# ACMMM2021-Anonymous/video-graph-ssl

Hardware: AMD Instinct MI355X
Metric: pretrain_clips_per_sec (higher is better)
Workload: dtype bf16x6 (fp32 tensors; conv products as 6 bf16 MFMAs on hi/mid/lo splits = fp32-grade, fp32 accumulate; everything else fp32)

## Files before the change

video-graph-ssl_amd/_hip.py:

```python
import ctypes as C
import os

import torch

_HERE = os.path.dirname(os.path.abspath(__file__))
LIB_PATH = os.environ.get('GCA_LIB_PATH') or os.path.join(_HERE, 'libgca_hip.so')


class HipLibraryMissing(RuntimeError):
    pass


if not os.path.exists(LIB_PATH):
    raise HipLibraryMissing(
        'libgca_hip.so is not built (%s). Run ./build_hip.sh or __graft_entry__.build(); there is no '
        'CPU fallback for the product path.' % LIB_PATH)
lib = C.CDLL(LIB_PATH)

c_i32, c_i64, c_f32, c_f64, c_vp = C.c_int32, C.c_int64, C.c_float, C.c_double, C.c_void_p


class ConvGeom(C.Structure):
    _fields_ = [(n, c_i32) for n in ('N', 'C', 'D', 'H', 'W', 'K', 'kd', 'kh', 'kw', 'sd', 'sh', 'sw',
                                     'pd', 'ph', 'pw', 'OD', 'OH', 'OW')] + [('x_batch_stride', c_i64)] + \
# ... 71 lines not shown
                                  c_f32, c_vp, c_vp, c_vp]),
    'gca_graph_gcn_fwd': (c_i32, [c_vp, c_vp, c_i64, c_i64, c_i64, c_i64, c_vp, c_vp]),
    'gca_graph_gcn_bwd_ws_bytes': (c_i64, [c_i64, c_i64, c_i64, c_i64]),
    'gca_graph_gcn_bwd': (c_i32, [c_vp, c_vp, c_vp, c_i64, c_i64, c_i64, c_i64, c_vp, c_vp, c_vp, c_vp]),
    'gca_ema_update': (c_i32, [c_vp, c_vp, c_i64, c_f32, c_vp]),
    'gca_ema_update_dev': (c_i32, [c_vp, c_vp, c_i64, c_vp, c_vp]),
    'gca_sgd_step': (c_i32, [c_vp, c_vp, c_vp, c_i64, c_vp, c_vp, c_f32, c_f32, c_i32, c_i32, c_vp, c_vp]),
    'gca_lars_job_chunks': (c_i32, []),
    'gca_lars_step': (c_i32, [c_vp, c_vp, c_vp, c_i64, c_vp, c_vp, c_vp, c_i64, c_vp, c_vp, c_i64, c_vp, c_vp, c_vp, c_vp, c_f32,
                              c_i32, c_f64, c_f64, c_vp, c_vp]),
    'gca_adam_step': (c_i32, [c_vp, c_vp, c_vp, c_vp, c_i64, c_vp, c_vp, c_f64, c_f64, c_f64, c_i32, c_vp, c_vp, c_vp]),
    'gca_adam_advance': (c_i32, [c_vp, c_vp, c_vp]),
    'gca_grad_clip_ws_bytes': (c_i64, []),
    'gca_grad_clip_coef': (c_i32, [c_vp, c_i64, c_f32, c_vp, c_vp, c_vp]),
    'gca_conv_wgrad_partial': (c_i32, [_GP, c_vp, c_vp, c_vp, c_vp, c_vp, c_vp, c_vp, c_vp]),
    'gca_conv_xf_ok': (c_i32, [_GP]),
    'gca_conv_fwd_xf': (c_i32, [_GP, c_vp, c_vp, c_vp, c_vp, c_vp, c_vp, c_vp, c_vp, c_vp, c_vp, c_vp]),
    'gca_conv_wgrad_xf': (c_i32, [_GP, c_vp, c_vp, c_vp, c_vp, c_vp, c_vp, c_i32, c_vp, c_vp]),
    'gca_conv_fwd_slabs': (c_i32, [_GP, c_vp, c_vp, c_vp, c_vp, c_vp, c_vp]),
    'gca_bn_train_fwd_slabs': (c_i32, [c_vp, c_i64, c_f64, c_vp, c_vp, c_f32, c_f32, c_vp, c_vp, c_vp, c_vp, c_vp, c_vp, c_vp, c_vp,
                                       c_vp, c_i32, c_i64, c_i64, c_i64, c_vp, c_i64, c_vp]),
    'gca_conv_dzf_ok': (c_i32, [_GP]),
    'gca_conv_wgrad_dzf': (c_i32, [_GP, c_vp, c_vp, c_vp, c_vp, c_i32, c_vp, c_vp, c_i32, c_vp, c_vp]),
    'gca_conv_wgrad_dzf_partial': (c_i32, [_GP, c_vp, c_vp, c_vp, c_vp, c_i32, c_vp, c_vp, c_vp, c_vp]),
    'gca_bn_bwd_consts_elems': (c_i64, [c_i64]),
    'gca_bn_bwd_sums': (c_i32, [c_vp, c_vp, c_vp, c_vp, c_vp, c_i32, c_i64, c_i64, c_i64, c_vp, c_vp, c_i64, c_vp, c_vp, c_vp,
                                c_vp, c_i32, c_vp]),
    'gca_reduce_jobs_finalize_host': (c_i64, [c_vp, c_i64]),
    'gca_splitk_reduce_batched': (c_i32, [c_vp, c_i64, c_i64, c_vp]),
    'gca_clip_prepare': (c_i32, [c_vp, c_i64, c_i64, c_i64, c_i64, c_i64, c_vp, c_vp, c_vp, c_i64, c_i64, c_vp, c_i32, c_vp]),
    'gca_clip_augment_ws_bytes': (c_i64, [c_i64, c_i64, c_i64]),
    'gca_clip_augment': (c_i32, [c_vp, c_i64, c_i64, c_i64, c_i64, c_i64, c_vp, c_vp, c_vp, c_vp, c_vp, c_vp, c_vp, c_i64, c_i64,
                                 c_vp, c_i32, c_vp, c_vp]),
    'gca_clip_views': (c_i32, [c_vp, c_i64, c_i64, c_i64, c_i64, c_vp, c_vp, c_i64, c_vp, c_i64, c_i64, c_i64, c_vp, c_vp, c_i64, c_i64,
                               c_i64, c_vp, c_vp]),
    'gca_retrieval_ws_bytes': (c_i64, [c_i64, c_i64, c_i64, c_i32, c_i32]),
    'gca_retrieval_topk': (c_i32, [c_vp, c_vp, c_i64, c_i64, c_i64, c_i32, c_i32, c_vp, c_vp, c_i32, c_vp, c_vp, c_vp, c_vp,
                                   c_i64, c_vp]),
    'gca_knn_vote': (c_i32, [c_vp, c_vp, c_i64, c_i32, c_i32, c_vp, c_i64, c_vp, c_i64, c_i64, c_i32, c_f32, c_vp, c_vp, c_vp,
                             c_vp]),
    'gca_ntxent_ws_bytes': (c_i64, [c_i64, c_i64]),
    'gca_ntxent_path': (c_i32, [c_i64, c_i64, c_i32, c_vp, c_vp]),
    'gca_ntxent_fwd': (c_i32, [c_vp, c_i64, c_i64, c_f32, c_vp, c_vp, c_vp, c_vp, c_vp, c_vp]),
    'gca_ntxent_bwd': (c_i32, [c_vp, c_vp, c_i64, c_i64, c_f32, c_vp, c_f32, c_vp, c_vp, c_vp]),
    'gca_barlow_ws_bytes': (c_i64, [c_i64, c_i64]),
    'gca_barlow_fwd': (c_i32, [c_vp, c_vp, c_i64, c_i64, c_f32, c_f32, c_vp, c_vp, c_vp, c_vp, c_vp, c_vp]),
    'gca_barlow_bwd': (c_i32, [c_vp, c_vp, c_vp, c_vp, c_vp, c_i64, c_i64, c_f32, c_vp, c_f32, c_vp, c_vp, c_vp, c_vp]),
    'gca_vicreg_ws_bytes': (c_i64, [c_i64, c_i64]),
    'gca_vicreg_fwd': (c_i32, [c_vp, c_vp, c_i64, c_i64, c_f32, c_f32, c_f32, c_f32, c_vp, c_vp, c_vp, c_vp, c_vp]),
    'gca_vicreg_bwd': (c_i32, [c_vp, c_vp, c_vp, c_vp, c_i64, c_i64, c_f32, c_f32, c_f32, c_vp, c_f32, c_vp, c_vp, c_vp, c_vp]),
    'gca_rows_normalize': (c_i32, [c_vp, c_i64, c_i64, c_vp]),
    'gca_swav_ws_bytes': (c_i64, [c_i64, c_i64, c_i64]),
    'gca_swav_fwd': (c_i32, [c_vp, c_vp, c_vp, c_i64, c_i64, c_i64, c_f32, c_f32, c_i64, c_vp, c_vp, c_vp, c_vp, c_vp]),
    'gca_swav_dz_splits': (c_i32, [c_i64, c_i64, c_i64]),
    'gca_swav_bwd': (c_i32, [c_vp, c_vp, c_vp, c_vp, c_i64, c_i64, c_i64, c_vp, c_f32, c_vp, c_vp, c_vp, c_i32, c_vp, c_vp]),
    'gca_dino_ws_bytes': (c_i64, [c_i64, c_i64, c_i64]),
    'gca_dino_fwd': (c_i32, [c_vp, c_vp, c_vp, c_vp, c_vp, c_vp, c_i64, c_i64, c_i64, c_f32, c_vp, c_f32, c_vp, c_i32, c_vp, c_vp, c_vp,
                             c_vp, c_vp]),
    'gca_dino_fwd_grid': (c_i32, [c_vp, c_vp, c_vp, c_vp, c_vp, c_vp, c_i64, c_i64, c_i64, c_f32, c_vp, c_f32, c_vp, c_i32, c_vp, c_vp,
                                  c_vp, c_i32, c_vp, c_vp]),
    'gca_classifier_ws_bytes': (c_i64, [c_i64, c_i64, c_i64]),
    'gca_classifier_fwd': (c_i32, [c_vp, c_vp, c_vp, c_vp, c_i64, c_i64, c_i64, c_vp, c_vp, c_vp, c_vp, c_vp, c_i64, c_vp]),
    'gca_classifier_bwd': (c_i32, [c_vp, c_vp, c_vp, c_vp, c_vp, c_vp, c_f32, c_i64, c_i64, c_i64, c_vp, c_vp, c_i32, c_vp, c_i32,
                                   c_vp, c_i64, c_vp]),
    'gca_rank_ge': (c_i32, [c_vp, c_vp, c_i64, c_i64, c_vp, c_vp]),
    'gca_grad_unscale_clip': (c_i32, [c_vp, c_i64, c_f32, c_vp, c_f32, c_f32, c_i32, c_f32, c_vp, c_vp, c_vp]),
    'gca_scale_dev': (c_i32, [c_vp, c_i64, c_vp, c_f32, c_vp]),
    'gca_fill': (c_i32, [c_vp, c_i64, c_f32, c_vp]),
    'gca_axpy': (c_i32, [c_vp, c_vp, c_i64, c_f32, c_vp]),
    'gca_scale': (c_i32, [c_vp, c_i64, c_f32, c_vp]),
    'gca_axpy_f16': (c_i32, [c_vp, c_vp, c_i64, c_f32, c_vp]),
    'gca_cast_f16': (c_i32, [c_vp, c_i64, c_i64, c_i64, c_vp, c_vp]),
    'gca_conv_pack_jobs_host': (c_i64, [_GP, c_i32, c_vp, c_vp, c_vp]),
    'gca_conv_pack_jobs_finalize_host': (c_i64, [c_vp, c_i64]),
    'gca_conv_pack_batched': (c_i32, [c_vp, c_i64, c_i64, c_vp]),
    'gca_gather_rows': (c_i32, [c_vp, c_vp, c_i64, c_i64, c_i64, c_vp, c_vp]),
}
for _name, (_res, _args) in SIGNATURES.items():
    _fn = getattr(lib, _name)
    _fn.restype, _fn.argtypes = _res, _args


PACK_JOB_BYTES = 128


class ReduceJob(C.Structure):
    _fields_ = [('slabs', C.c_void_p), ('dw', C.c_void_p), ('n', C.c_int64), ('splits', C.c_int32), ('accumulate', C.c_int32),
                ('first_block', C.c_int32), ('nblocks', C.c_int32)]


def ptr(t, half_ok=False):
    if t is None:
        return None
    if not t.is_cuda:
        raise RuntimeError('gca HIP ops need tensors on the GPU (got %s); there is no CPU fallback' % t.device)
    if t.dtype is not torch.float32 and not (half_ok and t.dtype is torch.float16) and t.is_floating_point():
        raise TypeError('this gca HIP op has no %s kernel' % t.dtype)
    return t.data_ptr()


def aptr(t):
    return ptr(t, True)


def is_half(*ts):
    kinds = {t.dtype for t in ts if t is not None}
    if len(kinds) > 1:
        raise TypeError('mixed activation storage types: %s' % sorted(map(str, kinds)))
    return int(kinds == {torch.float16})


def stream():
    return torch.cuda.current_stream().cuda_stream


def check(rc, what):
    if rc != 0:
        raise RuntimeError('%s failed with status %d (%s)' % (what, rc, {-1: 'invalid argument', -2: 'launch error'}.get(rc, '?')))


def call(name, *args):
    check(getattr(lib, name)(*args), name)
```

video-graph-ssl_amd/csrc/conv3d.hip:

```cpp
#include <cstring>
#include <type_traits>
#include "conv_halo.h"

#include <cstdlib>
#include <vector>

using namespace gca_conv;

namespace {

constexpr int LDK = BK + 4;
constexpr int lds_pitch(int math) { return math == 2 ? 28 : (math == 3 ? 12 : LDK); }
constexpr int lds_bufs(int tm, bool vec, int math) { return (math >= 1 || vec || tm >= 4) ? 1 : 2; }
constexpr int cmax(int a, int b) { return a > b ? a : b; }

template <int TM, int BN, int FAST, bool VEC, int MATH, bool H = false>
__device__ __forceinline__ void igemm_tile(
    const void* __restrict__ src, const float* __restrict__ apack, const int2* __restrict__ table,
    const float* __restrict__ bias, void* __restrict__ dst, float* __restrict__ psum,
    float* __restrict__ psq, float* __restrict__ slab, const IgemmParams p, int bid,
    float* __restrict__ As_, float* __restrict__ Bs_, int* __restrict__ taptab) {
  constexpr unsigned ES = H ? 2u : 4u;
  constexpr int BM = 32 * TM, TN = BN / 128;
  constexpr int A_F4 = (BM * 4 + 255) / 256;
// ... 585 lines not shown
                                      gca_xcd_remap((int)blockIdx.x - nA, (int)gridDim.x - nA), As_, Bs_, taptab);
  }
}

__device__ __forceinline__ int class_of(const int* __restrict__ first, int id) {
  int ci = 0;
#pragma unroll
  for (int i = 1; i < MAX_MERGED_CLASSES; ++i) ci += id >= first[i] ? 1 : 0;
  return ci;
}

template <int TM, int BN, int FAST, bool VEC, int MATH, bool H = false>
__global__ __launch_bounds__(256) void conv_igemm_classes_kernel(
    const void* __restrict__ src, const float* __restrict__ apack, const int2* __restrict__ table, void* __restrict__ dst,
    float* __restrict__ slab, const ClassBlock cb) {
  __shared__ __attribute__((aligned(16))) float As_[lds_bufs(TM, VEC, MATH) * 32 * TM * lds_pitch(MATH)];
  __shared__ __attribute__((aligned(16))) float Bs_[lds_bufs(TM, VEC, MATH) * BN * lds_pitch(MATH)];
  __shared__ int taptab[64];
  const int ci = class_of(cb.first_wg, (int)blockIdx.x);
  const int first = cb.first_wg[ci], count = cb.first_wg[ci + 1] - first;
  igemm_tile<TM, BN, FAST, VEC, MATH, H>(src, apack + cb.pack_off[ci], table + cb.table_off[ci], nullptr, dst, nullptr, nullptr,
                                         slab + cb.slab_off[ci], cb.p[ci], gca_xcd_remap((int)blockIdx.x - first, count), As_, Bs_,
                                         taptab);
}

constexpr int FINISH_CHUNK = 1024;
template <typename T>
__device__ __forceinline__ void splitk_finish_part(
    const float* __restrict__ slab, int splits, const float* __restrict__ bias, T* __restrict__ dst,
    float* __restrict__ psum, float* __restrict__ psq, const IgemmParams& p, int m, int part, int P, double* sh) {
  const float b = bias ? bias[m] : 0.f;
  const long long lo = (long long)part * FINISH_CHUNK;
  long long hi = lo + FINISH_CHUNK; if (hi > p.Ntot) hi = p.Ntot;
  const int QSP = p.QD * p.QH * p.QW, QHW = p.QH * p.QW, DHW = p.DH * p.DW;
  const long long DSP = (long long)p.DD * DHW;
  double s = 0.0, q = 0.0;
  for (long long n = lo + threadIdx.x; n < hi; n += 256) {
    float v = 0.f;
    const float* sp0 = slab + (long long)m * p.Ntot + n;
    const long long sstride = (long long)p.DK * p.Ntot;
    int k = 0;
    for (; k + 4 <= splits; k += 4) {
      const float l0 = sp0[(long long)k * sstride], l1 = sp0[(long long)(k + 1) * sstride];
      const float l2 = sp0[(long long)(k + 2) * sstride], l3 = sp0[(long long)(k + 3) * sstride];
      v += l0; v += l1; v += l2; v += l3;
    }
    for (; k < splits; ++k) v += sp0[(long long)k * sstride];
    s += (double)v; q += (double)v * (double)v;
    v += b;
    const int img = (int)(n / QSP);
    const int sp = (int)(n - (long long)img * QSP);
    const int qd = sp / QHW, rr = sp - qd * QHW;
    const int qh = rr / p.QW, qw = rr - qh * p.QW;
    const long long dsp = (long long)(qd * p.dm_d + p.do_d) * DHW + (qh * p.dm_h + p.do_h) * p.DW + (qw * p.dm_w + p.do_w);
    T* d = dst + ((long long)img * p.DK + m) * DSP + dsp;
    if (p.accumulate) v += (float)*d;
    *d = (T)v;
  }
  if (psum) {
    s = gca_block_sum256_d(s, sh);
    q = gca_block_sum256_d(q, sh);
    if (threadIdx.x == 0) { psum[(long long)m * P + part] = (float)s; psq[(long long)m * P + part] = (float)q; }
  }
}

template <typename T>
__global__ __launch_bounds__(256) void conv_splitk_finish_kernel(
    const float* __restrict__ slab, int splits, const float* __restrict__ bias, T* __restrict__ dst,
    float* __restrict__ psum, float* __restrict__ psq, IgemmParams p) {
  __shared__ double sh[4];
  splitk_finish_part<T>(slab, splits, bias, dst, psum, psq, p, blockIdx.x, blockIdx.y, gridDim.y, sh);
}

template <typename T>
__global__ __launch_bounds__(256) void conv_splitk_finish_classes_kernel(const float* __restrict__ slab, T* __restrict__ dst,
                                                                         const ClassBlock cb) {
  __shared__ double sh[4];
  const int ci = class_of(cb.first_part, (int)blockIdx.y);
  const int first = cb.first_part[ci];
  splitk_finish_part<T>(slab + cb.slab_off[ci], cb.p[ci].splits, nullptr, dst, nullptr, nullptr, cb.p[ci], blockIdx.x,
                        (int)blockIdx.y - first, cb.first_part[ci + 1] - first, sh);
}

__device__ __forceinline__ void pack_elements(const float* __restrict__ w, float* __restrict__ packed,
                                              const PackParams& p, long long first, long long step, long long end) {
  for (long long i = first; i < end; i += step) {
    const int m = (int)(i / p.Kpad), k = (int)(i - (long long)m * p.Kpad);
    float v = 0.f;
    if (m < p.M && k < p.Kred) {
      const int ch = k / p.ntaps, tl = k - ch * p.ntaps;
      const int a = tl / (p.nb * p.nc), r = tl - a * (p.nb * p.nc), b = r / p.nc, c = r - b * p.nc;
      const int tap = ((p.k0d + p.sd * a) * p.KH + (p.k0h + p.sh * b)) * p.KW + (p.k0w + p.sw * c);
      v = w[(long long)ch * p.s_ch + tap + (long long)m * p.s_m];
    }
    packed[i] = v;
  }
}
__global__ void conv_pack_kernel(const float* __restrict__ w, float* __restrict__ packed, PackParams p) {
  if (p.fmt >= 1)
    pack_halo_elements(w, reinterpret_cast<unsigned char*>(packed), p, (long long)blockIdx.x * blockDim.x + threadIdx.x,
                       (long long)gridDim.x * blockDim.x, pack_items(p));
  else
    pack_elements(w, packed, p, (long long)blockIdx.x * blockDim.x + threadIdx.x, (long long)gridDim.x * blockDim.x,
                  pack_items(p));
}

constexpr int PACK_CHUNK = 2048;
struct PackJob {
  PackParams p;
  const float* w;
  float* packed;
  int first_block, nblocks;
};
static_assert(sizeof(PackJob) <= GCA_PACK_JOB_BYTES, "gca_hip.h: GCA_PACK_JOB_BYTES too small");
__global__ __launch_bounds__(256) void conv_pack_batched_kernel(const unsigned char* __restrict__ jobs, int njobs) {
  const int bid = blockIdx.x;
  int lo = 0, hi = njobs - 1;
  while (lo < hi) {
    const int mid = (lo + hi + 1) >> 1;
    if (reinterpret_cast<const PackJob*>(jobs + (size_t)mid * GCA_PACK_JOB_BYTES)->first_block <= bid) lo = mid;
    else hi = mid - 1;
  }
  const PackJob* j = reinterpret_cast<const PackJob*>(jobs + (size_t)lo * GCA_PACK_JOB_BYTES);
  const PackParams p = j->p;
  const long long base = (long long)(bid - j->first_block) * PACK_CHUNK;
  long long end = base + PACK_CHUNK;
  const long long total = pack_items(p);
  if (end > total) end = total;
  if (p.fmt >= 1) pack_halo_elements(j->w, reinterpret_cast<unsigned char*>(j->packed), p, base + threadIdx.x, 256, end);
  else pack_elements(j->w, j->packed, p, base + threadIdx.x, 256, end);
}

__global__ void zero_fill_kernel(unsigned* __restrict__ p, long long n32, int tail16) {
  for (long long i = (long long)blockIdx.x * blockDim.x + threadIdx.x; i < n32; i += (long long)gridDim.x * blockDim.x) p[i] = 0u;
  if (tail16 && blockIdx.x == 0 && threadIdx.x == 0) reinterpret_cast<unsigned short*>(p + n32)[0] = 0;
}

enum class ConvKernel { Gather = 0, Halo = 1, Stem = 2, Pointwise = 3 };

struct IgemmCfg {
  int bm; int bn; int splits; int kt_per_split; int tail_bm; int main_cols; int math;
  ConvKernel kernel;
  int bd, bh, bw;
  int h;
};

inline int split_k(long long tiles, int nk, long long M, long long Ntot, int force, int& per) {
  int s = 1;
  if (force > 0) s = force;
  else if (tiles < 2 * NUM_CU && nk >= 8 && M * Ntot <= (1LL << 20)) {
    long long want = gca_ceil_div(2 * NUM_CU, tiles);
    if (want > nk / 4) want = nk / 4;
    if (want > 16) want = 16;
    if (want > 1) s = (int)want;
  }
  if (s > nk) s = nk;
  if (s < 1) s = 1;
  per = (int)gca_ceil_div(nk, s);
  return (int)gca_ceil_div(nk, per);
}

inline IgemmCfg choose_cfg(int M, long long Ntot, int nk, bool vec_ok, int force_bm, int force_splits) {
  IgemmCfg best{64, 128, 1, nk, 0, 0, 0, ConvKernel::Gather, 0, 0, 0, 0};
  double best_cost = 1e300;
  const bool force_vec = force_bm >= 1024;
  const int force_rows = force_bm & 1023;
  for (int v = 0; v < 2; ++v) {
    if (v == 1 && !vec_ok) continue;
    if (force_bm && (v == 1) != (force_vec && vec_ok)) continue;
    for (int tm = 1; tm <= 5; ++tm) {
      const int bm = 32 * tm, bn = v ? 256 : 128;
      if (force_rows && bm != force_rows) continue;
      const long long tiles = gca_ceil_div(M, bm) * gca_ceil_div(Ntot, bn);
      int per;
      const int s = split_k(tiles, nk, M, Ntot, force_splits, per);
      const double wg_per_cu = (double)(tiles * s) / NUM_CU;
      const double occ = wg_per_cu < 1.0 ? 0.55 : (wg_per_cu < 2.0 ? 0.75 : 1.0);
      const double rounds = (double)gca_ceil_div(tiles * s, NUM_CU);
      const double eff = (0.55 + 0.1 * tm) * (v ? 1.15 : 1.0) * occ;
      const double work = (double)bm * bn * per;
      const double cost = rounds * work / eff + (s > 1 ? 0.05 * rounds * work + 8.0 * bm * bn : 0.0);
      if (cost < best_cost) { best_cost = cost; best = IgemmCfg{bm, bn, s, per, 0, 0, 0, ConvKernel::Gather, 0, 0, 0, 0}; }
    }
  }
  return best;
}

inline void tune_of(const gca_conv_geom* g, int which, int& fbm, int& fs, int& tail, int& box) {
  if (which == 0) { fbm = g->tune_fwd_bm; fs = g->tune_fwd_splits; tail = g->tune_fwd_tail; box = g->tune_fwd_box; }
  else { fbm = g->tune_dgrad_bm; fs = g->tune_dgrad_splits; tail = g->tune_dgrad_tail; box = g->tune_dgrad_box; }
}

inline bool halo_heuristic_on() {
  static int on = -1;
  if (on < 0) { const char* e = getenv("GCA_HALO"); on = (e && e[0] == '0') ? 0 : 1; }
  return on != 0;
}
inline int ilog2(int v) { int l = 0; while ((1 << l) < v) ++l; return l; }
inline bool is_pow2(int v) { return v > 0 && (v & (v - 1)) == 0; }

inline bool pw_heuristic_on() {
  static int on = -1;
  if (on < 0) { const char* e = getenv("GCA_PW"); on = (e && e[0] == '0') ? 0 : 1; }
  return on != 0;
}
inline bool pw_geometry(const gca_conv_geom* g, int which, const IgemmParams& ip, PwParams& pw) {
  if (!g->act_f16 || g->kd != 1 || g->kh != 1 || g->kw != 1 || g->sd != 1 || g->sh != 1 || g->sw != 1 || g->pd || g->ph || g->pw)
    return false;
  const long long SP = (long long)g->D * g->H * g->W;
  if (SP % 8 != 0 || SP < 128 || g->x_batch_stride % 8 != 0) return false;
  const int Kc = which == 0 ? g->C : g->K, DK = which == 0 ? g->K : g->C;
  pw.DK = DK; pw.Kc = Kc; pw.Kpad = (int)gca_round_up(Kc, 32);
  pw.SP = (int)SP; pw.N = g->N;
// ... 476 lines not shown

int gca_version(void) { return 15; }

int gca_set_conv_math(int mode) {
  if (mode < 0 || mode > 2) return GCA_EINVAL;
  g_conv_math = mode;
  return GCA_OK;
}
int gca_get_conv_math(void) { return conv_math(); }

int64_t gca_conv_pack_elems(const gca_conv_geom* g, int which) {
  if (!geom_ok(g) || (which != 0 && which != 1)) return GCA_EINVAL;
  int64_t n = 0;
  for (const ClassInfo& c : resolve_launch(g, which).cls) n += pack_reserve(c);
  return n > 0 ? n : 64;
}

static void pack_params_of(const gca_conv_geom* g, int which, const ClassInfo& c, const IgemmCfg& cf, PackParams& p) {
  const int T = taps(g);
  p.fmt = (int)cf.kernel; p.math = cf.math; p.SC = c.srcC;
  p.nsteps = cf.kernel == ConvKernel::Stem ? cf.kt_per_split : cdiv(c.srcC, 16) * c.ntaps;
  const bool pwfmt = p.fmt == 3;
  p.Kred = (int)c.Kred; p.M = c.M; p.Kpad = pwfmt ? (int)gca_round_up(c.srcC, 32) : (int)c.Kpad; p.Mrows = pack_rows(c.M);
  p.ntaps = p.fmt == 2 ? g->kd * g->kh : c.ntaps; p.nb = c.nb; p.nc = c.nc;
  p.k0d = c.k0[0]; p.k0h = c.k0[1]; p.k0w = c.k0[2]; p.sd = c.ks[0]; p.sh = c.ks[1]; p.sw = c.ks[2];
  p.KH = g->kh; p.KW = g->kw; p.T = T;
  if (which == 0) { p.s_ch = T; p.s_m = (long long)g->C * T; }
  else { p.s_ch = (long long)g->C * T; p.s_m = T; }
}

int64_t gca_conv_pack_jobs_host(const gca_conv_geom* g, int which, const float* w, float* packed, void* jobs_out) {
  if (!geom_ok(g) || (which != 0 && which != 1)) return GCA_EINVAL;
  const ConvLaunch L = resolve_launch(g, which);
  int64_t n = 0;
  for (size_t i = 0; i < L.cls.size(); ++i) {
    const ClassInfo& c = L.cls[i];
    if (c.ntaps == 0) continue;
    if (jobs_out) {
      if (!w || !packed) return GCA_EINVAL;
      PackJob j{};
      pack_params_of(g, which, c, L.cf[i], j.p);
      j.w = w; j.packed = packed + c.pack_off;
      j.first_block = 0;
      j.nblocks = (int)gca_ceil_div(pack_items(j.p), PACK_CHUNK);
      unsigned char* dst = reinterpret_cast<unsigned char*>(jobs_out) + (size_t)n * GCA_PACK_JOB_BYTES;
      memset(dst, 0, GCA_PACK_JOB_BYTES);
      memcpy(dst, &j, sizeof(j));
    }
    ++n;
  }
  return n;
}

int64_t gca_conv_pack_jobs_finalize_host(void* jobs, int64_t njobs) {
  if (!jobs || njobs <= 0) return GCA_EINVAL;
  int64_t first = 0;
  for (int64_t i = 0; i < njobs; ++i) {
    PackJob j;
    unsigned char* rec = reinterpret_cast<unsigned char*>(jobs) + (size_t)i * GCA_PACK_JOB_BYTES;
    memcpy(&j, rec, sizeof(j));
    if (j.nblocks <= 0 || first + j.nblocks > 0x7fffffffLL) return GCA_EINVAL;
    j.first_block = (int)first;
    first += j.nblocks;
    memcpy(rec, &j, sizeof(j));
  }
  return first;
}

int gca_conv_pack_batched(const void* jobs_dev, int64_t njobs, int64_t total_blocks, void* stream) {
  if (!jobs_dev || njobs <= 0 || total_blocks <= 0 || total_blocks > 0x7fffffffLL) return GCA_EINVAL;
  hipLaunchKernelGGL(conv_pack_batched_kernel, dim3((unsigned)total_blocks), dim3(256), 0, (hipStream_t)stream,
                     reinterpret_cast<const unsigned char*>(jobs_dev), (int)njobs);
  return gca_launch_status();
}

int gca_conv_pack(const gca_conv_geom* g, int which, const float* w, float* packed, void* stream) {
  if (!geom_ok(g) || (which != 0 && which != 1) || !w || !packed) return GCA_EINVAL;
  const ConvLaunch L = resolve_launch(g, which);
  for (size_t i = 0; i < L.cls.size(); ++i) {
    const ClassInfo& c = L.cls[i];
    if (c.ntaps == 0) continue;
    PackParams p{};
    pack_params_of(g, which, c, L.cf[i], p);
    long long blocks = gca_ceil_div(pack_items(p), 256);
    if (blocks > 2048) blocks = 2048;
    hipLaunchKernelGGL(conv_pack_kernel, dim3((unsigned)blocks), dim3(256), 0, (hipStream_t)stream, w,
                       packed + c.pack_off, p);
  }
  return gca_launch_status();
}

int64_t gca_conv_table_rows(const gca_conv_geom* g, int which) {
  if (!geom_ok(g) || which < 0 || which > 2) return GCA_EINVAL;
  if (which == 2) return gca_round_up((int64_t)g->C * taps(g) + TABLE_PAD_W, 64);
  int64_t n = 0;
  for (const ClassInfo& c : resolve_launch(g, which).cls) if (c.ntaps) n += c.Kpad + 32;
  return n > 0 ? n : 32;
}

int gca_conv_table_build_host(const gca_conv_geom* g, int which, int32_t* t) {
  if (!geom_ok(g) || which < 0 || which > 2 || !t) return GCA_EINVAL;
  const int64_t HW = (int64_t)g->H * g->W, DHW = HW * g->D;
  if (which == 2) {
    const int T = taps(g);
    const int64_t rows = gca_conv_table_rows(g, 2), kred = (int64_t)g->C * T;
    for (int64_t k = 0; k < rows; ++k) {
      int32_t off = 0, pk = pack_row_meta(0, 0, 0, 0, 63);
      if (k < kred) {
        const int ch = (int)(k / T), tap = (int)(k % T);
        const int a = tap / (g->kh * g->kw), r = tap % (g->kh * g->kw), b = r / g->kw, c = r % g->kw;
        off = (int32_t)(uint32_t)((uint64_t)((ch * DHW + a * HW + (int64_t)b * g->W + c) * 4) & 0xffffffffu);
        pk = pack_row_meta(a, b, c, 1, tap < 63 ? tap : 63);
      }
      t[2 * k] = off; t[2 * k + 1] = pk;
    }
    return GCA_OK;
  }
  const ConvLaunch L = resolve_launch(g, which);
  const int64_t SHW = which == 0 ? HW : (int64_t)g->OH * g->OW;
  const int64_t SW = which == 0 ? g->W : g->OW;
  const int64_t SDHW = which == 0 ? DHW : SHW * g->OD;
  for (const ClassInfo& c : L.cls) {
    if (c.ntaps == 0) continue;
    int32_t* rows = t + 2 * c.table_off;
    for (int64_t k = 0; k < c.Kpad; ++k) {
      int32_t off = 0, pk = pack_row_meta(0, 0, 0, 0, 63);
      if (k < c.Kred) {
        const int ch = (int)(k / c.ntaps), tl = (int)(k % c.ntaps);
        const int a = tl / (c.nb * c.nc), r = tl % (c.nb * c.nc), b = r / c.nc, cc = r % c.nc;
        const int dd = c.dl0[0] + c.dls[0] * a, dh = c.dl0[1] + c.dls[1] * b, dw = c.dl0[2] + c.dls[2] * cc;
        off = (int32_t)(uint32_t)((uint64_t)((int64_t)(ch * SDHW + dd * SHW + dh * SW + dw) * 4) & 0xffffffffu);
        pk = pack_row_meta(dd, dh, dw, 1, tl < 63 ? tl : 63);
      }
      rows[2 * k] = off; rows[2 * k + 1] = pk;
    }
    int32_t* tt = rows + 2 * c.Kpad;
    for (int tl = 0; tl < 64; ++tl) {
      int32_t pk = 0;
      if (tl < c.ntaps && c.ntaps <= FAST_MAX_TAPS) {
        const int a = tl / (c.nb * c.nc), r = tl % (c.nb * c.nc), b = r / c.nc, cc = r % c.nc;
        pk = pack_row_meta(c.dl0[0] + c.dls[0] * a, c.dl0[1] + c.dls[1] * b, c.dl0[2] + c.dls[2] * cc, 1, 0);
      }
      tt[tl] = pk;
    }
  }
  return GCA_OK;
}

int64_t gca_conv_pack_layout(const gca_conv_geom* g, int which) {
  if (!geom_ok(g) || which < 0 || which > 1) return GCA_EINVAL;
  const ConvLaunch L = resolve_launch(g, which);
  int64_t sig = 0;
  for (const IgemmCfg& cf : L.cf) {
    int code = 0;
    switch (cf.kernel) {
      case ConvKernel::Gather: break;
      case ConvKernel::Halo: code = 4 + cf.math; break;
      case ConvKernel::Stem: code = cf.math; break;
      case ConvKernel::Pointwise: code = 8; break;
    }
    sig = sig * 16 + code;
    if (sig > (1LL << 56)) sig %= 1000000007LL;
  }
  return sig;
}

int gca_conv_kernel_cfg(const gca_conv_geom* g, int which, int32_t* out4) {
  if (!geom_ok(g) || which < 0 || which > 1 || !out4) return GCA_EINVAL;
// ... 124 lines not shown
```

video-graph-ssl_amd/csrc/conv_halo.h:

```cpp
#pragma once
#include "conv_igemm_host.h"

namespace gca_conv {

struct HaloParams {
  IgemmParams g;
  int bd, bh, bw;
  int lbh, lbw;
  int hd, hh, hw;
  int h0d, h0h, h0w;
  int dmin_d, dmin_h, dmin_w;
  int nbd, nbh, nbw;
  int P;
  int nchunks, chunks_per_split;
  int Mrows;
  unsigned cs_bytes;
  unsigned pack_bytes;
  const float* in_scale;
  const float* in_shift;
};

struct HaloCfg {
  int bm, bn;
  int bd, bh, bw;
  int splits, chunks_per_split;
  int math;
};

struct StemParams {
  IgemmParams g;
  int wm;
  int bd, bh, bw, lbh, lbw;
  int nbd, nbh, nbw;
  int hd, hh;
  int wp;
  int cd, hrowb;
  int sd, sh, pd, ph, pw;
  int kd, kh, kw;
  int nrows, nsteps;
  int Mrows;
  int rowoff_bytes;
  unsigned cs_bytes;
  unsigned pack_bytes;
  gca_magic m_w2, m_hdh, m_hh;
};

__device__ __forceinline__ void pack_halo_elements(const float* __restrict__ w, unsigned char* __restrict__ packed,
                                                   const PackParams& p, long long first, long long step, long long end) {
  if (p.fmt == 3) {
    const int kp2 = p.Kpad >> 1;
    for (long long i = first; i < end; i += step) {
      const int m = (int)(i / kp2), k = 2 * (int)(i - (long long)m * kp2);
      float v0 = 0.f, v1 = 0.f;
      if (m < p.M) {
        if (k < p.SC) v0 = w[(long long)k * p.s_ch + (long long)m * p.s_m];
        if (k + 1 < p.SC) v1 = w[(long long)(k + 1) * p.s_ch + (long long)m * p.s_m];
      }
      const unsigned lo = __builtin_bit_cast(unsigned short, (_Float16)v0), hi = __builtin_bit_cast(unsigned short, (_Float16)v1);
      reinterpret_cast<unsigned*>(packed)[i] = lo | (hi << 16);
    }
    return;
  }
  const int rowbytes = p.math == 3 ? 32 : (p.math == 2 ? 96 : 64);
  for (long long i = first; i < end; i += step) {
    const int kp = (int)(i & 7);
    const long long rowi = i >> 3;
    const int m = (int)(rowi % p.Mrows);
    const int s = (int)(rowi / p.Mrows);
    const int chunk = s / p.ntaps, tl = s - chunk * p.ntaps;
    const int a = tl / (p.nb * p.nc), r = tl - a * (p.nb * p.nc), b = r / p.nc, c = r - b * p.nc;
    const int tap = ((p.k0d + p.sd * a) * p.KH + (p.k0h + p.sh * b)) * p.KW + (p.k0w + p.sw * c);
    float v0 = 0.f, v1 = 0.f;
    const int ch = chunk * 16 + 2 * kp;
    if (p.fmt == 2) {
      const int rho = 2 * s + (kp >> 2), e0 = 2 * (kp & 3);
      if (m < p.M && rho < p.SC * p.ntaps) {
        const int c = rho / p.ntaps, ab = rho - c * p.ntaps;
        const int t0 = e0 < 4 ? 2 * e0 : 2 * (e0 - 4) + 1, t1 = e0 + 1 < 4 ? 2 * (e0 + 1) : 2 * (e0 + 1 - 4) + 1;
        const float* wr = w + (long long)c * p.s_ch + (long long)ab * p.KW + (long long)m * p.s_m;
        if (t0 < p.KW) v0 = wr[t0];
        if (t1 < p.KW) v1 = wr[t1];
      }
    } else if (m < p.M) {
      if (ch < p.SC) v0 = w[(long long)ch * p.s_ch + tap + (long long)m * p.s_m];
      if (ch + 1 < p.SC) v1 = w[(long long)(ch + 1) * p.s_ch + tap + (long long)m * p.s_m];
    }
    unsigned char* row = packed + rowi * rowbytes;
    if (p.math == 3) {
      const unsigned lo = __builtin_bit_cast(unsigned short, (_Float16)v0), hi = __builtin_bit_cast(unsigned short, (_Float16)v1);
      *reinterpret_cast<unsigned*>(row + 4 * kp) = lo | (hi << 16);
    } else if (p.math == 0) {
      *reinterpret_cast<float2*>(row + 8 * kp) = make_float2(v0, v1);
    } else if (p.math == 2) {
      unsigned h, md, l;
      split_bf16x3(v0, v1, h, md, l);
      *reinterpret_cast<unsigned*>(row + 4 * kp) = h;
      *reinterpret_cast<unsigned*>(row + 32 + 4 * kp) = md;
      *reinterpret_cast<unsigned*>(row + 64 + 4 * kp) = l;
    } else {
      unsigned h, l;
      split_bf16x2(v0, v1, h, l);
      *reinterpret_cast<unsigned*>(row + 4 * kp) = h;
      *reinterpret_cast<unsigned*>(row + 32 + 4 * kp) = l;
    }
  }
}

struct PwParams {
  int DK, Kc, Kpad;
  int SP, N;
  int tilesM, tiles_sp;
  int P;
  int accumulate;
  unsigned src_nstride;
  unsigned src_bytes, dst_bytes, pack_bytes;
};
int pw_launch(const PwParams& p, const void* src, const unsigned char* apack, const float* bias, void* dst, float* psum,
              float* psq, hipStream_t st);

size_t stem_lds_bytes(const StemParams& sp, int math);
int stem_launch(int math, const StemParams& sp, const void* src, const unsigned char* apack, const float* bias, void* dst,
                float* psum, float* psq, hipStream_t st);

inline int halo_row_bytes(int math) { return math == 3 ? 32 : (math == 2 ? 96 : 64); }
size_t halo_lds_bytes(int bm, int math, int P);
int halo_max_positions();
int halo_launch(const HaloCfg& c, const HaloParams& hp, const void* src, const unsigned char* apack, const int* tapdelta,
                const float* bias, void* dst, float* psum, float* psq, float* slab, hipStream_t st);

}
```

video-graph-ssl_amd/engine/layers.py:

```python
import math

import torch
import torch.nn as nn

from . import ops
from . import tape as _tape
from .tape import LazyVar, Var


GRAD_LOG = None


def _grad_of(p):
    if p.grad is None:
        p.grad = torch.zeros_like(p.data)
    if GRAD_LOG is not None:
        GRAD_LOG.append((_tape.CURRENT[0], p))
    return p.grad


class _PackedWeight(object):

    def _init_pack(self):
        self._pack, self._pack_plan, self._prepacked = [None, None], [None, None], [False, False]
        self._pack_layout = [None, None]

    def packed(self, plan, which):
        if self._prepacked[which] and self._pack_plan[which] is plan:
            if ops.H.lib.gca_conv_pack_layout(plan.gp, which) != self._pack_layout[which]:
                raise RuntimeError('packed weights are in a stale layout for this plan; rebuild the BatchedPacker')
            return self._pack[which]
        self._pack[which] = ops.conv_pack(plan, which, self.weight.data, self._pack[which])
        self._pack_plan[which] = plan
        self._pack_layout[which] = ops.H.lib.gca_conv_pack_layout(plan.gp, which)
        return self._pack[which]


class BatchedPacker(object):

    def __init__(self, module, directions):
        import ctypes
        H = ops.H
        recs, self.layers = [], []
        dev = None
        for m in module.modules():
            if not isinstance(m, _PackedWeight):
                continue
            for which in directions:
                plan, buf = m._pack_plan[which], m._pack[which]
                if plan is None or buf is None:
                    continue
                n = H.lib.gca_conv_pack_jobs_host(plan.gp, which, None, None, None)
                if n <= 0:
                    raise RuntimeError('gca_conv_pack_jobs_host: %d' % n)
                raw = ctypes.create_string_buffer(int(n) * H.PACK_JOB_BYTES)
                if H.lib.gca_conv_pack_jobs_host(plan.gp, which, m.weight.data_ptr(), buf.data_ptr(), raw) != n:
                    raise RuntimeError('gca_conv_pack_jobs_host failed')
                recs.append(raw.raw)
                m._pack_layout[which] = H.lib.gca_conv_pack_layout(plan.gp, which)
                self.layers.append((m, which, plan, buf))
                dev = buf.device
        blob = ctypes.create_string_buffer(b''.join(recs))
        self.n = (len(blob) - 1) // H.PACK_JOB_BYTES
        self.jobs, self.blocks = None, 0
        if self.n:
            self.blocks = H.lib.gca_conv_pack_jobs_finalize_host(blob, self.n)
            if self.blocks <= 0:
                raise RuntimeError('gca_conv_pack_jobs_finalize_host: %d' % self.blocks)
            self.jobs = torch.frombuffer(bytearray(blob.raw[:self.n * H.PACK_JOB_BYTES]), dtype=torch.uint8).to(dev)

    def run(self):
        if not self.n:
            return
        for m, which, plan, buf in self.layers:
            if m._pack[which] is not buf or m._pack_plan[which] is not plan:
                raise RuntimeError('BatchedPacker is stale (a layer was re-planned); rebuild it')
            m._prepacked[which] = True
        ops.H.call('gca_conv_pack_batched', ops.ptr(self.jobs), self.n, self.blocks, ops.stream())

    def release(self):
        for m, which, _, _ in self.layers:
            m._prepacked[which] = False


class HipConv3d(nn.Module, _PackedWeight):

    def __init__(self, cin, cout, kernel_size, stride=1, padding=0, bias=False):
        super().__init__()
        t3 = lambda v: (v, v, v) if isinstance(v, int) else tuple(v)
        self.in_channels, self.out_channels = cin, cout
        self.kernel_size, self.stride, self.padding = t3(kernel_size), t3(stride), t3(padding)
        self.weight = nn.Parameter(torch.empty(cout, cin, *self.kernel_size))
        self.bias = nn.Parameter(torch.empty(cout)) if bias else None
        nn.init.kaiming_uniform_(self.weight, a=math.sqrt(5))
        if bias:
            bound = 1 / math.sqrt(cin * self.kernel_size[0] * self.kernel_size[1] * self.kernel_size[2])
            nn.init.uniform_(self.bias, -bound, bound)
        self._init_pack()

    def plan(self, x):
        xs = 0
        if not x.is_contiguous():
            N, Cc, D, Hh, W = x.shape
            if x.stride()[1:] != (D * Hh * W, Hh * W, W, 1):
                raise RuntimeError('conv input must be NCDHW-contiguous inside each clip')
            xs = x.stride(0)
        return ops.conv_plan(tuple(x.shape), self.out_channels, self.kernel_size, self.stride, self.padding,
                             x.device, xs, act_f16=x.dtype is torch.float16)

    def forward(self, x):
        return ops.conv_fwd(self.plan(x), x, self.packed(self.plan(x), 0), None if self.bias is None else self.bias.data)


class _HipBatchNorm(nn.Module):
    def __init__(self, num_features, eps=1e-5, momentum=0.1, affine=True):
        super().__init__()
        self.num_features, self.eps, self.momentum = num_features, eps, momentum
        self.weight = nn.Parameter(torch.ones(num_features))
        self.bias = nn.Parameter(torch.zeros(num_features))
        self.register_buffer('running_mean', torch.zeros(num_features))
        self.register_buffer('running_var', torch.ones(num_features))
        self.register_buffer('num_batches_tracked', torch.tensor(0, dtype=torch.long))


class HipBatchNorm3d(_HipBatchNorm):
    pass


class HipBatchNorm1d(_HipBatchNorm):
    pass


class HipLinear(nn.Module, _PackedWeight):
    def __init__(self, fin, fout, bias=True):
        super().__init__()
        self.in_features, self.out_features = fin, fout
        self.weight = nn.Parameter(torch.empty(fout, fin))
        self.bias = nn.Parameter(torch.empty(fout)) if bias else None
        nn.init.kaiming_uniform_(self.weight, a=math.sqrt(5))
        if bias:
            bound = 1 / math.sqrt(fin)
            nn.init.uniform_(self.bias, -bound, bound)
# ... 417 lines not shown
```

Baseline: 1682.

## Route weight packing through specialized row-copy, LDS-tiled and fast-divide paths

Reworks the conv weight pack kernels so each block handles a fixed chunk and picks a route. Whole-kernel layouts become a vectorized float4 row copy, and layouts with s_m == T are transposed through an LDS tile with a tap lookup table. Other cases use float-reciprocal division in place of integer divides. The halo pack path gets the same reciprocal division, and the Python side adds a ctypes PackJob mirror and an eager repack when the layout changes. This targets the per-step weight repacking cost, in exchange for more code paths, float-division exactness limits guarded by PACK_FDIV_MAX, and extra shared memory per pack block.

```diff
diff --git a/video-graph-ssl_amd/_hip.py b/video-graph-ssl_amd/_hip.py
--- a/video-graph-ssl_amd/_hip.py
+++ b/video-graph-ssl_amd/_hip.py
@@ -177,6 +177,22 @@
 
 
 PACK_JOB_BYTES = 128
+PACK_CHUNK = 2048
+
+
+class PackJob(C.Structure):
+    _fields_ = [(n, C.c_int32) for n in ('Kred', 'M', 'Kpad', 'Mrows', 'ntaps', 'nb', 'nc', 'k0d', 'k0h', 'k0w', 'sd', 'sh', 'sw',
+                                         'KH', 'KW', 'T', 'fmt', 'SC', 'nsteps', 'math')] + [
+                ('s_ch', C.c_int64), ('s_m', C.c_int64), ('w', C.c_void_p), ('packed', C.c_void_p),
+                ('first_block', C.c_int32), ('nblocks', C.c_int32), ('_pad', C.c_ubyte * 8)]
+
+    def items(self):
+        if self.fmt == 3:
+            return self.Mrows * (self.Kpad >> 1)
+        return self.nsteps * self.Mrows * 8 if self.fmt >= 1 else self.Mrows * self.Kpad
+
+
+assert C.sizeof(PackJob) == PACK_JOB_BYTES
 
 
 class ReduceJob(C.Structure):
diff --git a/video-graph-ssl_amd/csrc/conv3d.hip b/video-graph-ssl_amd/csrc/conv3d.hip
--- a/video-graph-ssl_amd/csrc/conv3d.hip
+++ b/video-graph-ssl_amd/csrc/conv3d.hip
@@ -691,30 +691,135 @@
                         (int)blockIdx.y - first, cb.first_part[ci + 1] - first, sh);
 }
 
-__device__ __forceinline__ void pack_elements(const float* __restrict__ w, float* __restrict__ packed,
-                                              const PackParams& p, long long first, long long step, long long end) {
-  for (long long i = first; i < end; i += step) {
-    const int m = (int)(i / p.Kpad), k = (int)(i - (long long)m * p.Kpad);
+constexpr int PACK_CHUNK = 2048;
+constexpr int PACK_TILE_FLOATS = 4160;
+constexpr int PACK_TAB = 160;
+struct PackShared { float tile[PACK_TILE_FLOATS]; int tab[PACK_TAB]; };
+enum class PackRoute { Rows, Tile, Generic, Divide };
+
+__device__ __forceinline__ bool pack_aligned16(const void* q) { return (reinterpret_cast<size_t>(q) & 15) == 0; }
+__device__ __forceinline__ int pack_tile_rows(int T) { return T == 1 ? 64 : 32; }
+
+__device__ __forceinline__ PackRoute pack_route(const float* w, const float* packed, const PackParams& p) {
+  const long long total = pack_items(p);
+  if (total > 0x7fffffffLL || p.Kpad + PACK_CHUNK >= PACK_FDIV_MAX) return PackRoute::Divide;
+  const bool whole = p.ntaps == p.T && p.nb == p.KH && p.nc == p.KW && p.k0d == 0 && p.k0h == 0 && p.k0w == 0 && p.sd == 1 &&
+                     p.sh == 1 && p.sw == 1;
+  if (whole && p.s_ch == p.T && (p.Kred & 3) == 0 && (p.Kpad & 3) == 0 && (p.s_m & 3) == 0 && pack_aligned16(w) &&
+      pack_aligned16(packed))
+    return PackRoute::Rows;
+  if (p.s_m == p.T && ((pack_tile_rows(p.T) * p.T) | 1) <= PACK_TILE_FLOATS) return PackRoute::Tile;
+  return PackRoute::Generic;
+}
+
+template <bool FAST>
+__device__ __forceinline__ void pack_elements(const float* __restrict__ w, float* __restrict__ packed, const PackParams& p,
+                                              long long base, long long end) {
+  const int n = (int)(end - base), nbc = p.nb * p.nc;
+  const float inv_k = 1.0f / (float)p.Kpad, inv_taps = 1.0f / (float)p.ntaps, inv_bc = 1.0f / (float)nbc,
+              inv_c = 1.0f / (float)p.nc;
+  int m0, k0;
+  pack_split<FAST>(base, p.Kpad, m0, k0);
+  for (int li = threadIdx.x; li < n; li += 256) {
+    const int off = k0 + li, dm = pack_div<FAST>(off, p.Kpad, inv_k);
+    const int m = m0 + dm, k = off - dm * p.Kpad;
     float v = 0.f;
     if (m < p.M && k < p.Kred) {
-      const int ch = k / p.ntaps, tl = k - ch * p.ntaps;
-      const int a = tl / (p.nb * p.nc), r = tl - a * (p.nb * p.nc), b = r / p.nc, c = r - b * p.nc;
+      const int ch = pack_div<FAST>(k, p.ntaps, inv_taps), tl = k - ch * p.ntaps;
+      const int a = pack_div<FAST>(tl, nbc, inv_bc), r = tl - a * nbc, b = pack_div<FAST>(r, p.nc, inv_c), c = r - b * p.nc;
       const int tap = ((p.k0d + p.sd * a) * p.KH + (p.k0h + p.sh * b)) * p.KW + (p.k0w + p.sw * c);
       v = w[(long long)ch * p.s_ch + tap + (long long)m * p.s_m];
     }
-    packed[i] = v;
-  }
-}
-__global__ void conv_pack_kernel(const float* __restrict__ w, float* __restrict__ packed, PackParams p) {
-  if (p.fmt >= 1)
-    pack_halo_elements(w, reinterpret_cast<unsigned char*>(packed), p, (long long)blockIdx.x * blockDim.x + threadIdx.x,
-                       (long long)gridDim.x * blockDim.x, pack_items(p));
-  else
-    pack_elements(w, packed, p, (long long)blockIdx.x * blockDim.x + threadIdx.x, (long long)gridDim.x * blockDim.x,
-                  pack_items(p));
-}
-
-constexpr int PACK_CHUNK = 2048;
+    packed[base + li] = v;
+  }
+}
+
+__device__ __forceinline__ void pack_rows_copy(const float* __restrict__ w, float* __restrict__ packed, const PackParams& p,
+                                               long long base, long long end) {
+  const int n4 = (int)((end - base) >> 2), kp4 = p.Kpad >> 2, kr4 = p.Kred >> 2;
+  const float inv = 1.0f / (float)kp4;
+  int m0, k0;
+  pack_split<true>(base, p.Kpad, m0, k0);
+  float4* __restrict__ out = reinterpret_cast<float4*>(packed + base);
+  for (int f = threadIdx.x; f < n4; f += 256) {
+    const int off = (k0 >> 2) + f, dm = pack_div<true>(off, kp4, inv);
+    const int m = m0 + dm, k4 = off - dm * kp4;
+    float4 v = make_float4(0.f, 0.f, 0.f, 0.f);
+    if (m < p.M && k4 < kr4) v = *reinterpret_cast<const float4*>(w + (long long)m * p.s_m + 4 * k4);
+    out[f] = v;
+  }
+}
+
+__device__ __forceinline__ void pack_tiles(const float* __restrict__ w, float* __restrict__ packed, const PackParams& p,
+                                           unsigned blk, unsigned nblocks, PackShared& sh) {
+  const int tid = threadIdx.x, lane = tid & 63, wave = tid >> 6;
+  const int T = p.T, TM = pack_tile_rows(T), S = (TM * T) | 1;
+  const int TC = PACK_TILE_FLOATS / S < 64 ? PACK_TILE_FLOATS / S : 64;
+  const unsigned nct = (unsigned)((p.SC + TC - 1) / TC), ntiles = (unsigned)((p.M + TM - 1) / TM) * nct;
+  const int nbc = p.nb * p.nc;
+  for (unsigned t = blk; t < ntiles; t += nblocks) {
+    const unsigned mt = t / nct, ct = t - mt * nct;
+    const int m0 = (int)mt * TM, rows = p.M - m0 < TM ? p.M - m0 : TM;
+    const int c0 = (int)ct * TC, tc = p.SC - c0 < TC ? p.SC - c0 : TC;
+    const int nv = tc * p.ntaps, nk = nv + (ct == nct - 1 ? p.Kpad - p.Kred : 0);
+    __syncthreads();
+    if (tid < nk) {
+      int e = -1;
+      if (tid < nv) {
+        const int cl = tid / p.ntaps, tl = tid - cl * p.ntaps;
+        const int a = tl / nbc, r = tl - a * nbc, b = r / p.nc, c = r - b * p.nc;
+        e = cl * S + ((p.k0d + p.sd * a) * p.KH + (p.k0h + p.sh * b)) * p.KW + (p.k0w + p.sw * c);
+      }
+      sh.tab[tid] = e;
+    }
+    const int L = rows * T;
+    for (int cl = wave; cl < tc; cl += 4) {
+      const float* __restrict__ src = w + (long long)(c0 + cl) * p.s_ch + (long long)m0 * T;
+      for (int r = lane; r < L; r += 64) sh.tile[cl * S + r] = src[r];
+    }
+    __syncthreads();
+    int lg = 6;
+    if (nk <= 32) { lg = 0; while ((1 << lg) < nk) ++lg; }
+    const int width = 1 << lg, rpp = 64 >> lg;
+    float* __restrict__ dst = packed + (long long)m0 * p.Kpad + (long long)c0 * p.ntaps;
+    for (int r = wave * rpp + (lane >> lg); r < rows; r += 4 * rpp)
+      for (int kk = lane & (width - 1); kk < nk; kk += width) {
+        const int e = sh.tab[kk];
+        dst[(long long)r * p.Kpad + kk] = e < 0 ? 0.f : sh.tile[e + r * T];
+      }
+  }
+  const long long zb = (long long)p.M * p.Kpad, nz = (long long)(p.Mrows - p.M) * p.Kpad;
+  const long long first = (long long)blk * 256 + tid, step = (long long)nblocks * 256;
+  if ((nz & 3) == 0 && pack_aligned16(packed + zb)) {
+    float4* __restrict__ z = reinterpret_cast<float4*>(packed + zb);
+    for (long long i = first; i < (nz >> 2); i += step) z[i] = make_float4(0.f, 0.f, 0.f, 0.f);
+  } else {
+    for (long long i = first; i < nz; i += step) packed[zb + i] = 0.f;
+  }
+}
+
+__device__ __forceinline__ void pack_block(const float* __restrict__ w, float* __restrict__ packed, const PackParams& p,
+                                           unsigned blk, unsigned nblocks, PackShared& sh) {
+  const long long total = pack_items(p), base = (long long)blk * PACK_CHUNK;
+  const long long end = base + PACK_CHUNK < total ? base + PACK_CHUNK : total;
+  if (p.fmt >= 1) {
+    if (pack_halo_fast(p)) pack_halo_elements<true>(w, reinterpret_cast<unsigned char*>(packed), p, base, end);
+    else pack_halo_elements<false>(w, reinterpret_cast<unsigned char*>(packed), p, base, end);
+    return;
+  }
+  switch (pack_route(w, packed, p)) {
+    case PackRoute::Rows: pack_rows_copy(w, packed, p, base, end); break;
+    case PackRoute::Tile: pack_tiles(w, packed, p, blk, nblocks, sh); break;
+    case PackRoute::Generic: pack_elements<true>(w, packed, p, base, end); break;
+    default: pack_elements<false>(w, packed, p, base, end); break;
+  }
+}
+
+__global__ __launch_bounds__(256) void conv_pack_kernel(const float* __restrict__ w, float* __restrict__ packed, PackParams p) {
+  __shared__ PackShared sh;
+  pack_block(w, packed, p, blockIdx.x, gridDim.x, sh);
+}
+
 struct PackJob {
   PackParams p;
   const float* w;
@@ -723,6 +828,7 @@
 };
 static_assert(sizeof(PackJob) <= GCA_PACK_JOB_BYTES, "gca_hip.h: GCA_PACK_JOB_BYTES too small");
 __global__ __launch_bounds__(256) void conv_pack_batched_kernel(const unsigned char* __restrict__ jobs, int njobs) {
+  __shared__ PackShared sh;
   const int bid = blockIdx.x;
   int lo = 0, hi = njobs - 1;
   while (lo < hi) {
@@ -732,12 +838,7 @@
   }
   const PackJob* j = reinterpret_cast<const PackJob*>(jobs + (size_t)lo * GCA_PACK_JOB_BYTES);
   const PackParams p = j->p;
-  const long long base = (long long)(bid - j->first_block) * PACK_CHUNK;
-  long long end = base + PACK_CHUNK;
-  const long long total = pack_items(p);
-  if (end > total) end = total;
-  if (p.fmt >= 1) pack_halo_elements(j->w, reinterpret_cast<unsigned char*>(j->packed), p, base + threadIdx.x, 256, end);
-  else pack_elements(j->w, j->packed, p, base + threadIdx.x, 256, end);
+  pack_block(j->w, j->packed, p, (unsigned)(bid - j->first_block), (unsigned)j->nblocks, sh);
 }
 
 __global__ void zero_fill_kernel(unsigned* __restrict__ p, long long n32, int tail16) {
@@ -1380,8 +1481,8 @@
     if (c.ntaps == 0) continue;
     PackParams p{};
     pack_params_of(g, which, c, L.cf[i], p);
-    long long blocks = gca_ceil_div(pack_items(p), 256);
-    if (blocks > 2048) blocks = 2048;
+    const long long blocks = gca_ceil_div(pack_items(p), PACK_CHUNK);
+    if (blocks > 0x7fffffffLL) return GCA_EINVAL;
     hipLaunchKernelGGL(conv_pack_kernel, dim3((unsigned)blocks), dim3(256), 0, (hipStream_t)stream, w,
                        packed + c.pack_off, p);
   }
diff --git a/video-graph-ssl_amd/csrc/conv_halo.h b/video-graph-ssl_amd/csrc/conv_halo.h
--- a/video-graph-ssl_amd/csrc/conv_halo.h
+++ b/video-graph-ssl_amd/csrc/conv_halo.h
@@ -45,43 +45,70 @@
   gca_magic m_w2, m_hdh, m_hh;
 };
 
+constexpr int PACK_FDIV_MAX = 1 << 21;
+template <bool FAST>
+__device__ __forceinline__ int pack_div(int n, int d, float inv) {
+  return FAST ? (int)(((float)n + 0.5f) * inv) : n / d;
+}
+template <bool FAST>
+__device__ __forceinline__ void pack_split(long long base, int d, int& q, int& r) {
+  if (FAST) { const unsigned b = (unsigned)base; q = (int)(b / (unsigned)d); r = (int)(b - (unsigned)q * (unsigned)d); }
+  else { const long long qq = base / d; q = (int)qq; r = (int)(base - qq * d); }
+}
+__host__ __device__ inline bool pack_halo_fast(const PackParams& p) {
+  if (pack_items(p) > 0x7fffffffLL) return false;
+  if (p.fmt == 3) return (p.Kpad >> 1) + 2048 < PACK_FDIV_MAX;
+  return p.Mrows + 256 < PACK_FDIV_MAX && 2 * p.nsteps + 2 < PACK_FDIV_MAX;
+}
+
+template <bool FAST>
 __device__ __forceinline__ void pack_halo_elements(const float* __restrict__ w, unsigned char* __restrict__ packed,
-                                                   const PackParams& p, long long first, long long step, long long end) {
+                                                   const PackParams& p, long long base, long long end) {
+  const int n = (int)(end - base);
   if (p.fmt == 3) {
     const int kp2 = p.Kpad >> 1;
-    for (long long i = first; i < end; i += step) {
-      const int m = (int)(i / kp2), k = 2 * (int)(i - (long long)m * kp2);
+    const float inv = 1.0f / (float)kp2;
+    int m0, k0;
+    pack_split<FAST>(base, kp2, m0, k0);
+    for (int li = threadIdx.x; li < n; li += 256) {
+      const int off = k0 + li, dm = pack_div<FAST>(off, kp2, inv);
+      const int m = m0 + dm, k = 2 * (off - dm * kp2);
       float v0 = 0.f, v1 = 0.f;
       if (m < p.M) {
         if (k < p.SC) v0 = w[(long long)k * p.s_ch + (long long)m * p.s_m];
         if (k + 1 < p.SC) v1 = w[(long long)(k + 1) * p.s_ch + (long long)m * p.s_m];
       }
       const unsigned lo = __builtin_bit_cast(unsigned short, (_Float16)v0), hi = __builtin_bit_cast(unsigned short, (_Float16)v1);
-      reinterpret_cast<unsigned*>(packed)[i] = lo | (hi << 16);
+      reinterpret_cast<unsigned*>(packed)[base + li] = lo | (hi << 16);
     }
     return;
   }
   const int rowbytes = p.math == 3 ? 32 : (p.math == 2 ? 96 : 64);
-  for (long long i = first; i < end; i += step) {
-    const int kp = (int)(i & 7);
-    const long long rowi = i >> 3;
-    const int m = (int)(rowi % p.Mrows);
-    const int s = (int)(rowi / p.Mrows);
-    const int chunk = s / p.ntaps, tl = s - chunk * p.ntaps;
-    const int a = tl / (p.nb * p.nc), r = tl - a * (p.nb * p.nc), b = r / p.nc, c = r - b * p.nc;
-    const int tap = ((p.k0d + p.sd * a) * p.KH + (p.k0h + p.sh * b)) * p.KW + (p.k0w + p.sw * c);
+  const int nbc = p.nb * p.nc;
+  const float inv_rows = 1.0f / (float)p.Mrows, inv_taps = 1.0f / (float)p.ntaps, inv_bc = 1.0f / (float)nbc,
+              inv_c = 1.0f / (float)p.nc;
+  int s0, r0;
+  pack_split<FAST>(base >> 3, p.Mrows, s0, r0);
+  for (int li = threadIdx.x; li < n; li += 256) {
+    const int kp = li & 7;
+    const long long rowi = (base >> 3) + (li >> 3);
+    const int roff = r0 + (li >> 3), ds = pack_div<FAST>(roff, p.Mrows, inv_rows);
+    const int m = roff - ds * p.Mrows, s = s0 + ds;
     float v0 = 0.f, v1 = 0.f;
-    const int ch = chunk * 16 + 2 * kp;
     if (p.fmt == 2) {
       const int rho = 2 * s + (kp >> 2), e0 = 2 * (kp & 3);
       if (m < p.M && rho < p.SC * p.ntaps) {
-        const int c = rho / p.ntaps, ab = rho - c * p.ntaps;
+        const int c = pack_div<FAST>(rho, p.ntaps, inv_taps), ab = rho - c * p.ntaps;
         const int t0 = e0 < 4 ? 2 * e0 : 2 * (e0 - 4) + 1, t1 = e0 + 1 < 4 ? 2 * (e0 + 1) : 2 * (e0 + 1 - 4) + 1;
         const float* wr = w + (long long)c * p.s_ch + (long long)ab * p.KW + (long long)m * p.s_m;
         if (t0 < p.KW) v0 = wr[t0];
         if (t1 < p.KW) v1 = wr[t1];
       }
     } else if (m < p.M) {
+      const int chunk = pack_div<FAST>(s, p.ntaps, inv_taps), tl = s - chunk * p.ntaps;
+      const int a = pack_div<FAST>(tl, nbc, inv_bc), r = tl - a * nbc, b = pack_div<FAST>(r, p.nc, inv_c), c = r - b * p.nc;
+      const int tap = ((p.k0d + p.sd * a) * p.KH + (p.k0h + p.sh * b)) * p.KW + (p.k0w + p.sw * c);
+      const int ch = chunk * 16 + 2 * kp;
       if (ch < p.SC) v0 = w[(long long)ch * p.s_ch + tap + (long long)m * p.s_m];
       if (ch + 1 < p.SC) v1 = w[(long long)(ch + 1) * p.s_ch + tap + (long long)m * p.s_m];
     }
diff --git a/video-graph-ssl_amd/engine/layers.py b/video-graph-ssl_amd/engine/layers.py
--- a/video-graph-ssl_amd/engine/layers.py
+++ b/video-graph-ssl_amd/engine/layers.py
@@ -50,6 +50,9 @@
                 plan, buf = m._pack_plan[which], m._pack[which]
                 if plan is None or buf is None:
                     continue
+                layout = H.lib.gca_conv_pack_layout(plan.gp, which)
+                if m._pack_layout[which] != layout:
+                    ops.conv_pack(plan, which, m.weight.data, buf)
                 n = H.lib.gca_conv_pack_jobs_host(plan.gp, which, None, None, None)
                 if n <= 0:
                     raise RuntimeError('gca_conv_pack_jobs_host: %d' % n)
@@ -57,7 +60,7 @@
                 if H.lib.gca_conv_pack_jobs_host(plan.gp, which, m.weight.data_ptr(), buf.data_ptr(), raw) != n:
                     raise RuntimeError('gca_conv_pack_jobs_host failed')
                 recs.append(raw.raw)
-                m._pack_layout[which] = H.lib.gca_conv_pack_layout(plan.gp, which)
+                m._pack_layout[which] = layout
                 self.layers.append((m, which, plan, buf))
                 dev = buf.device
         blob = ctypes.create_string_buffer(b''.join(recs))
```

Result: no change. 1689 (median of 6 runs) (+0.4%).
